# dfki-asr/morphablegraphs

Hardware: AMD Instinct MI355X
Metric: motion-primitive samples scored+back-projected/sec; fraction of HBM roofline (higher is better)
Workload: dtype f32; 1 GPU; walk primitive L=40 F=156 D=79 NB=31 GMM k=8, batch=8192 candidates/GPU (BASELINE.json configs[1]); candidates_per_gpu=8192, global_candidates=8192, collective=none, clock_ramp_steps=1500

## Files before the change

include/mg_hip.h:

```cpp
#ifndef MG_HIP_H
#define MG_HIP_H

#include <stdint.h>

#ifdef __cplusplus
extern "C" {
#endif

typedef struct mg_context mg_context;
typedef struct mg_primitive mg_primitive;
typedef struct mg_time_grid mg_time_grid;
typedef struct mg_constraint_set mg_constraint_set;

enum {
    MG_OK = 0,
    MG_ERR_INVALID_ARGUMENT = -1,
    MG_ERR_NO_DEVICE = -2,
    MG_ERR_HIP = -3,
    MG_ERR_UNSUPPORTED = -4,
    MG_ERR_NOT_POSITIVE_DEFINITE = -5,
    MG_ERR_OUT_OF_MEMORY = -6
};

enum { MG_F32 = 0, MG_F64 = 1 };
// ... 81 lines not shown
#define MG_OPT_FORCE_VALU_SCORE 0
#define MG_OPT_FORCE_VALU_SAMPLE 1
#define MG_OPT_RING_SLOTS 2
#define MG_OPT_CHUNK_WINDOW 3
#define MG_OPT_CHUNK_SAMPLES 4
#define MG_OPT_FRAMES_KERNEL 5
#define MG_OPT_PLACED_FAST_PCT 6
#define MG_OPT_OPTIONS_STEP 7
#define MG_OPT_PLAIN_MALLOC 8
#define MG_OPT_GMM_KERNEL 9
#define MG_OPT_SCORE_KERNEL 10
#define MG_OPT_ROOT_MODE 11
#define MG_OPT_PLACED_HOLD 12
#define MG_OPT_TRAJECTORY_LANES 13
#define MG_OPT_TRAJECTORY_SEARCH 14
#define MG_OPT_COUNT 15
int mg_context_set_option(mg_context *ctx, int32_t option, int32_t value);
int mg_context_arena_begin(mg_context *ctx, int64_t block_bytes);
int mg_context_arena_end(mg_context *ctx);
int mg_context_arena_bytes(mg_context *ctx, int64_t *reserved, int64_t *used);
int mg_context_synchronize(mg_context *ctx);
int mg_context_device_info(mg_context *ctx, char *name, int32_t *n_cu, int64_t *total_mem);

int mg_device_malloc(mg_context *ctx, int64_t bytes, void **out_dev);
int mg_device_free(mg_context *ctx, void *ptr_dev);
int mg_context_trim_outputs(mg_context *ctx);
int mg_context_output_bytes(mg_context *ctx, int64_t *reserved, int64_t *in_use, int32_t *n_regions, int32_t *n_fast);
int mg_device_malloc_chunked(mg_context *ctx, int64_t bytes, int64_t chunk_bytes, void **out_dev);
int mg_device_malloc_placed(mg_context *ctx, int64_t bytes, int32_t max_candidates, void **out_dev, double *info4);
int mg_device_probe_placement(mg_context *ctx, void *buf_dev, int64_t bytes, double *info4);
int mg_device_placement_info(mg_context *ctx, const void *buf_dev, double *info4, double *tbps);
// ... 317 lines not shown
```

morphablegraphs_amd/_capi.py:

```python
import ctypes as C
import functools
import itertools
import os

import numpy as np

HERE = os.path.dirname(os.path.abspath(__file__))
LIB_PATH = os.path.join(HERE, "csrc", "libmg_hip.so")

MG_OK = 0
MG_ERR_INVALID_ARGUMENT = -1
MG_ERR_UNSUPPORTED = -4
MG_F32, MG_F64 = 0, 1
MG_PATH_AUTO, MG_PATH_MFMA, MG_PATH_DIRECT = 0, 1, 2
MG_ALIGN_START_POSE = -1
MG_OPT_FORCE_VALU_SCORE, MG_OPT_FORCE_VALU_SAMPLE, MG_OPT_RING_SLOTS, MG_OPT_CHUNK_WINDOW, MG_OPT_CHUNK_SAMPLES = 0, 1, 2, 3, 4
MG_OPT_FRAMES_KERNEL = 5
MG_OPT_PLACED_FAST_PCT = 6
MG_OPT_OPTIONS_STEP = 7
MG_OPT_PLAIN_MALLOC = 8
MG_OPT_GMM_KERNEL = 9
MG_OPT_SCORE_KERNEL = 10
MG_OPT_ROOT_MODE = 11
MG_OPT_PLACED_HOLD = 12
MG_OPT_TRAJECTORY_LANES = 13
MG_OPT_TRAJECTORY_SEARCH = 14
MG_OPT_COUNT = 15
MG_CONSTRAINT_POSITION, MG_CONSTRAINT_DIRECTION_2D, MG_CONSTRAINT_JOINT_POSITION = 0, 1, 2
MG_CONSTRAINT_JOINT_MIDPOINT, MG_CONSTRAINT_JOINT_ORIENTATION, MG_CONSTRAINT_LOOK_AT, MG_CONSTRAINT_POSE = 3, 4, 5, 6
MG_CONSTRAINT_VALUE_POSITION, MG_CONSTRAINT_VALUE_HEADING = 7, 8
PROFILE_SLOTS = {"frames": 0, "gmm_log_prob": 1, "score_constraints": 2, "argmin": 3,
                 "gmm_sample": 4, "spline_evaluate": 5, "step": 6, "options_step": 7, "joint_tracks": 8, "frame_constraints": 9, "trajectory": 10,
                 "cluster_tree_search": 11, "walk_frames": 12}
MG_TREE_MAX_DEPTH, MG_TREE_MAX_CHILDREN, MG_TREE_MAX_CANDIDATES = 64, 256, 64
MG_TREE_TIE, MG_TREE_NO_RESULT, MG_TREE_OVERFLOW, MG_TREE_NO_MEAN = 1, 2, 4, 8
MG_KD_MAX_DEPTH = 64
TREE_SEARCH_RECORD = np.dtype([("row", "<i8"), ("leaf", "<i4"), ("flags", "<i4"), ("evaluations", "<i8"), ("value", "<f8")])
MG_WALK_MAX_STEPS = 64
MG_WALK_TILE = 32
MG_FUSED_MAX_OPTIONS = 24


# ... 1470 lines not shown
```

morphablegraphs_amd/csrc/mg_gmm.hip:

```cpp
#include <cstring>

#include <algorithm>

#include "mg_internal.h"
#include "mg_gmm_device.h"
#include "mg_score_device.h"

#define MG_GMM_CANDS 64
#define MG_GMM_WAVES 8

struct mg_gmm_args {
    const double *P;
    const double *mP;
    const double *cst;
    const void *x;
    void *out;
    int64_t B, ld;
    int32_t K, L;
};

template <bool X_F64, bool OUT_F64>
__global__ __launch_bounds__(MG_GMM_CANDS *MG_GMM_WAVES) void mg_gmm_logp_kernel(mg_gmm_args a) {
    extern __shared__ __attribute__((aligned(16))) unsigned char smem[];
    const int L = a.L, K = a.K;
// ... 131 lines not shown
    for (int q = 0; q < MG_JAC_ITEMS; q++) {
        const int e = tid + 256 * q;
        if (e < MG_JAC_CANDS * L) {
            const int c = e / L, i = e - c * L;
            if (c < ncand)
                ((double *)a.out)[(b0 + c) * L + i] = (exp(lds_lp[c]) == 0.0) ? 1.0 : g[q];
        }
    }
}



struct mg_gmm_mfma_args {
    int64_t B, ld;
    int32_t K, L, JT;
};

template <int KK, bool X_F64, bool OUT_F64>
__global__ __launch_bounds__(256) void mg_gmm_logp_mfma_kernel(const double *__restrict__ Ppack,
                                                              const double *__restrict__ mP,
                                                              const double *__restrict__ cst,
                                                              const void *__restrict__ x, void *__restrict__ out,
                                                              const mg_gmm_mfma_args a) {
    extern __shared__ __attribute__((aligned(16))) unsigned char smem[];
    mg_lds_f64 *lds_t = (mg_lds_f64 *)smem;
    mg_lds_f64 *lds_e = lds_t + a.K * 16;
    const int tid = threadIdx.x, lane = tid & 63;
    const int wave = __builtin_amdgcn_readfirstlane(tid >> 6);
    const int cl = lane & 15, g = lane >> 4;
    const int64_t b0 = (int64_t)blockIdx.x * 16;
    const int ncand = (int)((a.B - b0) < 16 ? (a.B - b0) : 16);
    typename mg_gmm_xt<X_F64>::type xf[KK];
    mg_gmm_load_x<KK, X_F64>(xf, x, b0, ncand, a.ld, a.L, cl, g);
    for (int k = wave; k < a.K; k += 4) {
        mg_gmm_frag<KK> f;
        mg_gmm_load_component<KK>(f, Ppack, mP, cst, k, a.JT, lane, cl, a.K);
        mg_gmm_apply_component(f, k, a.JT, xf, lds_t, cl, g);
    }
    __syncthreads();
    for (int e = tid; e < a.K * 16; e += 256) lds_e[e] = mg_gmm_exp_entry(lds_t, a.K, e);
    __syncthreads();
    if (tid < ncand) {
        const double r = mg_gmm_logsumexp(lds_t, lds_e, a.K, tid);
        if (OUT_F64) ((double *)out)[b0 + tid] = r;
        else ((float *)out)[b0 + tid] = (float)r;
    }
}

template <int KK>
static int mg_launch_gmm_mfma_kk(mg_primitive *p, const void *x, int xdt, int64_t B, int64_t ld, void *out, int odt) {
    mg_gmm_mfma_args a;
    a.B = B; a.ld = ld; a.K = p->K; a.L = p->Lg; a.JT = (p->Lg + 15) / 16;
    const int64_t grid = (B + 15) / 16;
    if (grid > 0x7fffffff) { mg_set_error("mg_gmm_log_prob: too many samples"); return MG_ERR_UNSUPPORTED; }
    const size_t lds = (size_t)p->K * 16 * 8 * 2;
    hipStream_t st = p->ctx->stream;
    const bool xf = xdt == MG_F64, of = odt == MG_F64;
    if (xf && of) hipLaunchKernelGGL((mg_gmm_logp_mfma_kernel<KK, true, true>), dim3((int)grid), dim3(256), lds, st, p->d_gPpack, p->d_gmPpad, p->d_gconst, x, out, a);
    else if (xf) hipLaunchKernelGGL((mg_gmm_logp_mfma_kernel<KK, true, false>), dim3((int)grid), dim3(256), lds, st, p->d_gPpack, p->d_gmPpad, p->d_gconst, x, out, a);
    else if (of) hipLaunchKernelGGL((mg_gmm_logp_mfma_kernel<KK, false, true>), dim3((int)grid), dim3(256), lds, st, p->d_gPpack, p->d_gmPpad, p->d_gconst, x, out, a);
    else hipLaunchKernelGGL((mg_gmm_logp_mfma_kernel<KK, false, false>), dim3((int)grid), dim3(256), lds, st, p->d_gPpack, p->d_gmPpad, p->d_gconst, x, out, a);
    MG_HIP_CHECK(hipGetLastError());
    return MG_OK;
}

template <int KK>
__host__ __device__ constexpr int mg_gmm_nf() {
    int nf = 0;
    for (int jt = 0; jt < (KK + 3) / 4; jt++) nf += (4 * (jt + 1) < KK) ? 4 * (jt + 1) : KK;
    return nf;
}
struct mg_objective_args {
    mg_score_args sa;
    const double *Wpack, *bpad;
    int32_t RT, rows, wave_doubles;
    int32_t pair_doubles;
    double error_scale, quality_scale;
    double *err_out, *obj_out;
};
template <bool SCORE> struct mg_gmm_lds_nw { static constexpr int value = SCORE ? 12 : 16; };
template <int KK, bool X_F64, bool OUT_F64, bool SCORE>
__global__ __launch_bounds__(64 * mg_gmm_lds_nw<SCORE>::value) void mg_gmm_logp_lds_kernel(const double *__restrict__ Ppack,
                                                               const double *__restrict__ mP,
                                                               const double *__restrict__ cst,
                                                               const void *__restrict__ x, void *__restrict__ out,
                                                               const mg_gmm_mfma_args a, const int64_t n_tiles, const mg_objective_args oa) {
    constexpr int JTM = (KK + 3) / 4;
    constexpr int NW = mg_gmm_lds_nw<SCORE>::value;
    extern __shared__ __attribute__((aligned(16))) unsigned char smem[];
    const int K = a.K;
    constexpr int JT = JTM;
    constexpr int nf = mg_gmm_nf<KK>();
    mg_lds_f64 *lds_f = (mg_lds_f64 *)smem;
    mg_lds_f64 *lds_c = lds_f + (size_t)K * nf * 64;
    mg_lds_f64 *lds_w = lds_c + (size_t)K * JT * 16;
    const int tid = threadIdx.x, lane = tid & 63;
    const int wave = __builtin_amdgcn_readfirstlane(tid >> 6);
    const int cl = lane & 15, g = lane >> 4;
    typedef double mg_f64x2 __attribute__((ext_vector_type(2)));
    const mg_f64x2 *P2 = (const mg_f64x2 *)(Ppack + (size_t)K * JT * KK * 64);
#pragma unroll 4
    for (int F2 = wave; F2 < K * nf / 2; F2 += NW) {
        const int F = 2 * F2, k = F / nf, f = F - k * nf;
        int jt = 0, off = 0;
#pragma unroll
        for (int j = 0; j < JTM - 1; j++) {
            const int n = (4 * (j + 1) < KK) ? 4 * (j + 1) : KK;
            if (f >= off + n) { off += n; jt = j + 1; }
        }
        const mg_f64x2 v = P2[(((size_t)k * JT + jt) * (KK / 2) + (f - off) / 2) * 64 + lane];
        lds_f[F * 64 + lane] = v[0];
        lds_f[(F + 1) * 64 + lane] = v[1];
    }
    for (int e = tid; e < K * JT * 16; e += 64 * NW) lds_c[e] = -mP[e];
    __syncthreads();
    mg_lds_f64 *terms = lds_w + (size_t)wave * (SCORE ? oa.wave_doubles : 2 * K * 16), *exps = terms + K * 16;
    double *vals_b = SCORE && oa.pair_doubles > 0 ? (double *)(lds_w + (size_t)NW * oa.wave_doubles + (size_t)wave * oa.pair_doubles) : nullptr;
    bool pending = false;
    double r_a = 0.0;
    int64_t b0_a = 0;
    int ncand_a = 0;
    for (int64_t tile = (int64_t)wave * gridDim.x + blockIdx.x; tile < n_tiles; tile += (int64_t)gridDim.x * NW) {
        const int64_t b0 = tile * 16;
        const int ncand = (int)((a.B - b0) < 16 ? (a.B - b0) : 16);
        typename mg_gmm_xt<X_F64>::type xf[KK];
        mg_gmm_load_x<KK, X_F64>(xf, x, b0, ncand, a.ld, a.L, cl, g);
        for (int k = 0; k < K; k++) {
            __builtin_amdgcn_sched_barrier(0);
            const mg_lds_f64 *fk = lds_f + (size_t)k * nf * 64 + lane;
            mg_f64x4 acc[JTM];
#pragma unroll
            for (int jt = 0; jt < JTM; jt++) {
                const double c0 = lds_c[(k * JT + jt) * 16 + cl];
                acc[jt] = {c0, c0, c0, c0};
            }
#pragma unroll
            for (int kk = 0; kk < KK; kk++) {
                int off = 0;
#pragma unroll
                for (int jt = 0; jt < JTM; jt++) {
                    if (kk < 4 * (jt + 1)) acc[jt] = __builtin_amdgcn_mfma_f64_16x16x4f64((double)xf[kk], fk[(off + kk) * 64], acc[jt], 0, 0, 0);
                    off += (4 * (jt + 1) < KK) ? 4 * (jt + 1) : KK;
                }
            }
// ... 70 lines not shown
#define MG_GMM_LDS_MIN_B 20480
static int mg_objective_wave_doubles(const mg_primitive *p, const mg_constraint_set *cs) {
    return std::max(2 * p->K * 16, 16 * (cs->rows + 1) + 32 * std::max(cs->n, 1));
}
template <int KK>
static int mg_launch_gmm_lds_kk(mg_primitive *p, const void *x, int xdt, int64_t B, int64_t ld, void *out, int odt,
                                const mg_constraint_set *cs = nullptr, double error_scale = 0.0, double quality_scale = 0.0,
                                double *err_out = nullptr, double *obj_out = nullptr) {
    mg_gmm_mfma_args a;
    a.B = B; a.ld = ld; a.K = p->K; a.L = p->Lg; a.JT = (p->Lg + 15) / 16;
    const int64_t n_tiles = (B + 15) / 16;
    mg_objective_args oa;
    memset(&oa, 0, sizeof(oa));
    const int wave_doubles = cs ? mg_objective_wave_doubles(p, cs) : 2 * p->K * 16;
    const int nw = cs ? mg_gmm_lds_nw<true>::value : mg_gmm_lds_nw<false>::value;
    size_t lds = ((size_t)p->K * mg_gmm_lds_nf(KK, a.JT) * 64 + (size_t)p->K * a.JT * 16 + (size_t)nw * wave_doubles) * 8;
    const int pair_doubles = cs ? 16 * (cs->rows + 1) : 0;
    const bool pairs = cs && lds + (size_t)nw * pair_doubles * 8 <= 160 * 1024;
    if (pairs) lds += (size_t)nw * pair_doubles * 8;
    if (cs) {
        mg_score_args &sa = oa.sa;
        sa = mg_score_args_of(cs, p->L);
        sa.lat = x; sa.B = B; sa.ld = ld;
        oa.Wpack = cs->d_Wpack; oa.bpad = cs->d_bpad; oa.RT = cs->RT; oa.rows = cs->rows; oa.wave_doubles = wave_doubles;
        oa.pair_doubles = pairs ? pair_doubles : 0;
        oa.error_scale = error_scale; oa.quality_scale = quality_scale; oa.err_out = err_out; oa.obj_out = obj_out;
    }
    const int grid = (int)std::min<int64_t>(std::max(1, p->ctx->n_cu), n_tiles);
    hipStream_t st = p->ctx->stream;
    const bool xf = xdt == MG_F64, of = odt == MG_F64;
    const unsigned abit = 1u << (KK / 2);
    if (!(p->ctx->attr_gmm_lds & abit)) {
        MG_HIP_CHECK(hipFuncSetAttribute((const void *)mg_gmm_logp_lds_kernel<KK, true, true, false>, hipFuncAttributeMaxDynamicSharedMemorySize, 160 * 1024));
        MG_HIP_CHECK(hipFuncSetAttribute((const void *)mg_gmm_logp_lds_kernel<KK, true, false, false>, hipFuncAttributeMaxDynamicSharedMemorySize, 160 * 1024));
        MG_HIP_CHECK(hipFuncSetAttribute((const void *)mg_gmm_logp_lds_kernel<KK, false, true, false>, hipFuncAttributeMaxDynamicSharedMemorySize, 160 * 1024));
        MG_HIP_CHECK(hipFuncSetAttribute((const void *)mg_gmm_logp_lds_kernel<KK, false, false, false>, hipFuncAttributeMaxDynamicSharedMemorySize, 160 * 1024));
        MG_HIP_CHECK(hipFuncSetAttribute((const void *)mg_gmm_logp_lds_kernel<KK, true, true, true>, hipFuncAttributeMaxDynamicSharedMemorySize, 160 * 1024));
        MG_HIP_CHECK(hipFuncSetAttribute((const void *)mg_gmm_logp_lds_kernel<KK, false, true, true>, hipFuncAttributeMaxDynamicSharedMemorySize, 160 * 1024));
        p->ctx->attr_gmm_lds |= abit;
    }
    if (cs) {
        if (xf) hipLaunchKernelGGL((mg_gmm_logp_lds_kernel<KK, true, true, true>), dim3(grid), dim3(64 * nw), lds, st, p->d_gPpack, p->d_gmPpad, p->d_gconst, x, out, a, n_tiles, oa);
        else hipLaunchKernelGGL((mg_gmm_logp_lds_kernel<KK, false, true, true>), dim3(grid), dim3(64 * nw), lds, st, p->d_gPpack, p->d_gmPpad, p->d_gconst, x, out, a, n_tiles, oa);
    }
    else if (xf && of) hipLaunchKernelGGL((mg_gmm_logp_lds_kernel<KK, true, true, false>), dim3(grid), dim3(1024), lds, st, p->d_gPpack, p->d_gmPpad, p->d_gconst, x, out, a, n_tiles, oa);
    else if (xf) hipLaunchKernelGGL((mg_gmm_logp_lds_kernel<KK, true, false, false>), dim3(grid), dim3(1024), lds, st, p->d_gPpack, p->d_gmPpad, p->d_gconst, x, out, a, n_tiles, oa);
    else if (of) hipLaunchKernelGGL((mg_gmm_logp_lds_kernel<KK, false, true, false>), dim3(grid), dim3(1024), lds, st, p->d_gPpack, p->d_gmPpad, p->d_gconst, x, out, a, n_tiles, oa);
    else hipLaunchKernelGGL((mg_gmm_logp_lds_kernel<KK, false, false, false>), dim3(grid), dim3(1024), lds, st, p->d_gPpack, p->d_gmPpad, p->d_gconst, x, out, a, n_tiles, oa);
    MG_HIP_CHECK(hipGetLastError());
    return MG_OK;
}

bool mg_objective_can_fuse(const mg_primitive *p, const mg_constraint_set *cs) {
    if (!p->d_gPpack || p->KKg <= 0 || p->Lg != p->L || p->KK != p->KKg || !cs || !cs->d_Wpack || p->ctx->opt[MG_OPT_FORCE_VALU_SCORE]) return false;
    for (const mg_keyframe_constraint &kc : cs->structure)
        if (kc.type != MG_CONSTRAINT_POSITION && kc.type != MG_CONSTRAINT_DIRECTION_2D) return false;
    if (cs->has_pose || cs->align_joint > 0) return false;
    const int JT = (p->Lg + 15) / 16;
    if (JT != (p->KKg + 3) / 4) return false;
    const size_t lds = ((size_t)p->K * mg_gmm_lds_nf(p->KKg, JT) * 64 + (size_t)p->K * JT * 16 + (size_t)mg_gmm_lds_nw<true>::value * mg_objective_wave_doubles(p, cs)) * 8;
    return lds <= 160 * 1024 - 64;
}
int mg_launch_objective(mg_primitive *p, const mg_constraint_set *cs, const void *x, int xdt, int64_t B, int64_t ld, double error_scale,
// ... 440 lines not shown
```

morphablegraphs_amd/csrc/mg_gmm_device.h:

```cpp
#pragma once
#include <hip/hip_runtime.h>

#include <cmath>

typedef double mg_f64x4 __attribute__((ext_vector_type(4)));
typedef __attribute__((address_space(3))) double mg_lds_f64;
typedef __attribute__((address_space(3))) float mg_lds_f32;

template <bool X_F64> struct mg_gmm_xt { typedef double type; };
template <> struct mg_gmm_xt<false> { typedef float type; };

template <int KK, bool X_F64>
__device__ __forceinline__ void mg_gmm_load_x(typename mg_gmm_xt<X_F64>::type (&xf)[KK], const void *x, int64_t b0, int ncand,
                                              int64_t ld, int L, int cl, int g) {
    typedef typename mg_gmm_xt<X_F64>::type T;
    const int c = cl < ncand ? cl : ncand - 1;
    const bool rok = cl < ncand;
    const T *row = (const T *)x + (b0 + c) * ld;
    const T *rowg = row + g;
#pragma unroll
    for (int kk = 0; kk < KK; kk++) {
        if (kk < KK - 2) {
            const T v = rowg[4 * kk];
            xf[kk] = rok ? v : (T)0;
// ... 57 lines not shown
template <int JTM>
__device__ __forceinline__ void mg_gmm_finish_component(const mg_f64x4 (&acc)[JTM], int JT, double cst, int k, mg_lds_f64 *terms, int cl, int g) {
    double part[4] = {0.0, 0.0, 0.0, 0.0};
#pragma unroll
    for (int jt = 0; jt < JTM; jt++)
        if (jt < JT) {
#pragma unroll
            for (int r = 0; r < 4; r++) part[r] = fma(acc[jt][r], acc[jt][r], part[r]);
        }
#pragma unroll
    for (int r = 0; r < 4; r++) part[r] = mg_row16_sum(part[r]);
    if (cl == 0) {
#pragma unroll
        for (int r = 0; r < 4; r++) terms[k * 16 + g + 4 * r] = cst - 0.5 * part[r];
    }
}

template <int KK, typename T, bool WIDEN_AT_USE = false>
__device__ __forceinline__ void mg_gmm_apply_component(const mg_gmm_frag<KK> &f, int k, int JT, const T (&xf)[KK],
                                                       mg_lds_f64 *terms, int cl, int g) {
    constexpr int JTM = mg_gmm_frag<KK>::JTM;
    mg_f64x4 acc[JTM];
#pragma unroll
    for (int jt = 0; jt < JTM; jt++) acc[jt] = {f.c0[jt], f.c0[jt], f.c0[jt], f.c0[jt]};
#pragma unroll
    for (int kk = 0; kk < KK; kk++) {
        T xv = xf[kk];
        if constexpr (WIDEN_AT_USE) asm volatile("" : "+v"(xv));
        const double xd = (double)xv;
#pragma unroll
// ... 104 lines not shown
```

morphablegraphs_amd/csrc/mg_host.hip:

```cpp
#include <algorithm>
#include <cmath>
#include <cstdarg>
#include <cstdio>
#include <cstdlib>
#include <cstring>
#include <new>
#include <time.h>

#include "mg_internal.h"
#include <dlfcn.h>

static thread_local char g_err[1024] = "";

void mg_set_error(const char *fmt, ...) {
    va_list ap;
    va_start(ap, fmt);
    vsnprintf(g_err, sizeof(g_err), fmt, ap);
    va_end(ap);
}

int mg_hip_fail(hipError_t e, const char *what) {
    mg_set_error("HIP error %d (%s) in %s", (int)e, hipGetErrorString(e), what);
    if (e == hipErrorOutOfMemory) return MG_ERR_OUT_OF_MEMORY;
    if (e == hipErrorNoDevice || e == hipErrorInvalidDevice) return MG_ERR_NO_DEVICE;
// ... 80 lines not shown
        return MG_ERR_UNSUPPORTED;
    }
    if (stream) {
        ctx->stream = (hipStream_t)stream;
        ctx->own_stream = false;
    } else {
        e = hipStreamCreateWithFlags(&ctx->stream, hipStreamNonBlocking);
        if (e != hipSuccess) { delete ctx; return mg_hip_fail(e, "hipStreamCreate"); }
        ctx->own_stream = true;
    }
    e = hipMalloc(&ctx->argmin_out, 16);
    if (e != hipSuccess) { mg_context_destroy(ctx); return mg_hip_fail(e, "hipMalloc"); }
    int rc = mg_setup_kernel_attributes(ctx);
    if (rc == MG_OK) rc = mg_options_fused_attributes();
    if (rc != MG_OK) { mg_context_destroy(ctx); return rc; }
    *out = ctx;
    return MG_OK;
}

static void mg_vmm_release(mg_context *ctx, mg_context::vmm_alloc &v);
extern "C" void mg_context_destroy(mg_context *ctx) {
    if (!ctx) return;
    (void)hipSetDevice(ctx->device);
    (void)hipStreamSynchronize(ctx->stream);
    if (ctx->rccl_comm && g_rccl.CommDestroy) { (void)g_rccl.CommDestroy(ctx->rccl_comm); ctx->rccl_comm = nullptr; }
    for (auto &p : ctx->pending) { (void)hipEventDestroy(p.a); (void)hipEventDestroy(p.b); }
    for (auto &ev : ctx->free_events) (void)hipEventDestroy(ev);
    for (auto &st : ctx->side) if (st) (void)hipStreamDestroy(st);
    for (auto &e : ctx->side_ev) if (e) (void)hipEventDestroy(e);
    if (ctx->scratch) (void)mg_device_free(ctx, ctx->scratch);
// ... 147 lines not shown
    ctx->dist_rank = 0; ctx->dist_ranks = 1;
    return nrc == 0 ? MG_OK : mg_rccl_fail(nrc, "ncclCommDestroy");
}

extern "C" int mg_context_synchronize(mg_context *ctx) {
    MG_REQUIRE(ctx != nullptr, "mg_context_synchronize: ctx is NULL");
    MG_HIP_CHECK(hipStreamSynchronize(ctx->stream));
    return MG_OK;
}

extern "C" int mg_context_set_reserved_cus(mg_context *ctx, int32_t n) {
    MG_REQUIRE(ctx != nullptr && n >= 0, "mg_context_set_reserved_cus: bad arguments");
    ctx->reserved_cus = std::min<int32_t>(n, ctx->n_cu - 1);
    return MG_OK;
}
extern "C" int mg_context_set_option(mg_context *ctx, int32_t option, int32_t value) {
    MG_REQUIRE(ctx != nullptr, "mg_context_set_option: ctx is NULL");
    MG_REQUIRE(option >= 0 && option < MG_OPT_COUNT, "mg_context_set_option: unknown option %d", option);
    MG_REQUIRE(value >= 0, "mg_context_set_option: value %d < 0", value);
    ctx->opt[option] = value;
    return MG_OK;
}
extern "C" int mg_context_device_info(mg_context *ctx, char *name, int32_t *n_cu, int64_t *total_mem) {
    MG_REQUIRE(ctx != nullptr, "mg_context_device_info: ctx is NULL");
    if (name) { strncpy(name, ctx->name, 255); name[255] = 0; }
    if (n_cu) *n_cu = ctx->n_cu;
    if (total_mem) *total_mem = ctx->total_mem;
    return MG_OK;
}

// ... 440 lines not shown
extern "C" mg_time_grid *mg_primitive_canonical_grid(mg_primitive *prim) { return prim ? prim->canonical : nullptr; }
extern "C" int mg_time_grid_size(const mg_time_grid *g) { return g ? g->T : 0; }
extern "C" int mg_time_grid_get_tables(const mg_time_grid *g, int32_t *i0, double *weights, double *times) {
    MG_REQUIRE(g != nullptr, "mg_time_grid_get_tables: grid is NULL");
    if (i0) std::copy(g->i0.begin(), g->i0.end(), i0);
    if (weights) std::copy(g->w.begin(), g->w.end(), weights);
    if (times) std::copy(g->times.begin(), g->times.end(), times);
    return MG_OK;
}

static void mg_primitive_free(mg_primitive *p) {
    if (!p) return;
    (void)hipSetDevice(p->ctx->device);
    (void)hipStreamSynchronize(p->ctx->stream);
    void *ptrs[] = {p->d_Epack, p->d_Et32, p->d_Et64, p->d_Erpack, p->d_meanroot, p->d_mean32, p->d_mean, p->d_knots,
                    p->d_gP, p->d_gmP, p->d_gconst, p->d_gmean, p->d_gchol, p->d_gPpack, p->d_gmPpad, p->d_gPTpack, p->d_gcholpack, p->d_gmeanpad,
                    p->d_tphi, p->d_tmean};
    for (void *q : ptrs) mg_dev_free(p->ctx, q);
    for (mg_time_grid *g : {p->canonical, p->coeff_grid})
        if (g) { mg_free_grid_device(g); delete g; }
    delete p;
}

extern "C" void mg_primitive_destroy(mg_primitive *p) {
    if (p && p->ctx) p->ctx->fused_next.valid = false;
    mg_primitive_free(p);
}

extern "C" int mg_primitive_create(mg_context *ctx, const mg_primitive_desc *d, mg_primitive **out) {
    MG_REQUIRE(ctx && d && out, "mg_primitive_create: NULL argument");
    *out = nullptr;
// ... 197 lines not shown
            if (rc == MG_OK) rc = mg_upload(ctx, cpack, &p->d_gcholpack);
            if (rc == MG_OK) rc = mg_upload(ctx, meanpad, &p->d_gmeanpad);
            {
                const size_t n1 = ppack.size();
                ppack.resize(2 * n1, 0.0);
                for (int k = 0; k < K; k++)
                    for (int jt = 0; jt < JT; jt++)
                        for (int q = 0; q < KK / 2; q++)
                            for (int lane = 0; lane < 64; lane++)
                                for (int h = 0; h < 2; h++)
                                    ppack[n1 + ((((size_t)k * JT + jt) * (KK / 2) + q) * 64 + lane) * 2 + h] = ppack[((((size_t)k * JT + jt) * KK) + 2 * q + h) * 64 + lane];
            }
            if (rc == MG_OK) rc = mg_upload(ctx, ppack, &p->d_gPpack);
            if (rc == MG_OK) rc = mg_upload(ctx, ptpack, &p->d_gPTpack);
            if (rc == MG_OK) rc = mg_upload(ctx, mpad, &p->d_gmPpad);
        }
        if (rc == MG_OK) rc = mg_upload(ctx, gP, &p->d_gP);
        if (rc == MG_OK) rc = mg_upload(ctx, gmP, &p->d_gmP);
        if (rc == MG_OK) rc = mg_upload(ctx, gconst, &p->d_gconst);
        if (rc == MG_OK) rc = mg_upload(ctx, p->gm, &p->d_gmean);
        if (rc == MG_OK) rc = mg_upload(ctx, chol, &p->d_gchol);
        if (rc != MG_OK) { mg_primitive_free(p); return rc; }
    }

    {
        std::vector<double> m2(L, 1.0);
        double wsum = 0.0;
        for (int j = 0; j < K; j++) wsum += p->gw[j];
        if (K > 0)
            for (int k = 0; k < L; k++) {
// ... 1189 lines not shown
```

morphablegraphs_amd/csrc/mg_internal.h:

```cpp
#pragma once
#include <hip/hip_runtime.h>

#include <cstdint>
#include <map>
#include <string>
#include <vector>

#include "../../include/mg_hip.h"

#define MG_NCAND 16
#define MG_ROWTILE 16
#define MG_MAX_KK 16
#define MG_BLOCK 256
#define MG_PROFILE_SLOTS 13

void mg_set_error(const char *fmt, ...);
int mg_hip_fail(hipError_t e, const char *what);

#define MG_HIP_CHECK(expr)                                   \
    do {                                                     \
        hipError_t _e = (expr);                              \
        if (_e != hipSuccess) return mg_hip_fail(_e, #expr); \
    } while (0)

#define MG_REQUIRE_AS(cond, code, ...) \
    do {                               \
        if (!(cond)) {                 \
            mg_set_error(__VA_ARGS__); \
            return (code);             \
        }                              \
    } while (0)

struct mg_event_pair {
    hipEvent_t a, b;
    int slot;
    bool ended;
    int slot2 = -1;
};

struct mg_context {
    int device = 0;
    hipStream_t stream = nullptr;
    bool own_stream = false;
    int n_cu = 0;
    int64_t total_mem = 0;
    int max_lds = 0;
    char name[256] = {0};
    bool profile = false;
    std::vector<mg_event_pair> pending;
    std::vector<hipEvent_t> free_events;
    int reserved_cus = 0;
    int32_t opt[MG_OPT_COUNT] = {0};
    int prof_interval = 1;
// ... 119 lines not shown
    std::vector<double> knots;
    std::vector<double> gw, gm, gc, gp;
    int32_t Dp = 0;
    int32_t cshift = 0;
    float *d_Epack = nullptr;
    float *d_Et32 = nullptr;
    double *d_Et64 = nullptr;
    double *d_Erpack = nullptr;
    double *d_meanroot = nullptr;
    float *d_mean32 = nullptr;
    double *d_mean = nullptr;
    double *d_knots = nullptr;
    int32_t RRT = 0;
    double *d_gPpack = nullptr;
    double *d_gmPpad = nullptr;
    double *d_gP = nullptr;
    double *d_gmP = nullptr;
    double *d_gPTpack = nullptr;
    double *d_gcholpack = nullptr;
    double *d_gmeanpad = nullptr;
    double *d_gconst = nullptr;
    double *d_gmean = nullptr;
    double *d_gchol = nullptr;
    mg_time_grid *canonical = nullptr;
    mg_time_grid *coeff_grid = nullptr;
};

struct mg_constraint_set {
    mg_primitive *prim = nullptr;
    int32_t n = 0;
// ... 106 lines not shown
```

Before: 106.5 million samples/s.

## Pack half-empty last GMM precision tiles of component pairs into one MFMA tile

When the latent width leaves the last 16-column tile of each component's Cholesky-like precision matrix at most half full, a host-side image now packs two components' last tiles into one shared 16-wide tile. The MFMA and LDS GMM log-prob kernels then run a single MFMA chain for that tile per component pair and split the result with a DPP swap. This removes MFMA work and LDS fragment storage spent on zero-padded columns. The cost is extra index arithmetic in the fragment staging loop, more code paths, and one extra device buffer. It is enabled by default through a new context option.

```diff
diff --git a/include/mg_hip.h b/include/mg_hip.h
--- a/include/mg_hip.h
+++ b/include/mg_hip.h
@@ -119,7 +119,8 @@
 #define MG_OPT_PLACED_HOLD 12
 #define MG_OPT_TRAJECTORY_LANES 13
 #define MG_OPT_TRAJECTORY_SEARCH 14
-#define MG_OPT_COUNT 15
+#define MG_OPT_GMM_PACK_LAST 15
+#define MG_OPT_COUNT 16
 int mg_context_set_option(mg_context *ctx, int32_t option, int32_t value);
 int mg_context_arena_begin(mg_context *ctx, int64_t block_bytes);
 int mg_context_arena_end(mg_context *ctx);
diff --git a/morphablegraphs_amd/_capi.py b/morphablegraphs_amd/_capi.py
--- a/morphablegraphs_amd/_capi.py
+++ b/morphablegraphs_amd/_capi.py
@@ -25,7 +25,8 @@
 MG_OPT_PLACED_HOLD = 12
 MG_OPT_TRAJECTORY_LANES = 13
 MG_OPT_TRAJECTORY_SEARCH = 14
-MG_OPT_COUNT = 15
+MG_OPT_GMM_PACK_LAST = 15
+MG_OPT_COUNT = 16
 MG_CONSTRAINT_POSITION, MG_CONSTRAINT_DIRECTION_2D, MG_CONSTRAINT_JOINT_POSITION = 0, 1, 2
 MG_CONSTRAINT_JOINT_MIDPOINT, MG_CONSTRAINT_JOINT_ORIENTATION, MG_CONSTRAINT_LOOK_AT, MG_CONSTRAINT_POSE = 3, 4, 5, 6
 MG_CONSTRAINT_VALUE_POSITION, MG_CONSTRAINT_VALUE_HEADING = 7, 8
diff --git a/morphablegraphs_amd/csrc/mg_gmm.hip b/morphablegraphs_amd/csrc/mg_gmm.hip
--- a/morphablegraphs_amd/csrc/mg_gmm.hip
+++ b/morphablegraphs_amd/csrc/mg_gmm.hip
@@ -169,10 +169,14 @@
 struct mg_gmm_mfma_args {
     int64_t B, ld;
     int32_t K, L, JT;
+    int32_t pack;
 };
+
+static bool mg_gmm_pack_last(const mg_primitive *p) { return p->d_gPshare != nullptr && p->ctx->opt[MG_OPT_GMM_PACK_LAST] != 0; }
 
 template <int KK, bool X_F64, bool OUT_F64>
 __global__ __launch_bounds__(256) void mg_gmm_logp_mfma_kernel(const double *__restrict__ Ppack,
+                                                              const double *__restrict__ Pshare,
                                                               const double *__restrict__ mP,
                                                               const double *__restrict__ cst,
                                                               const void *__restrict__ x, void *__restrict__ out,
@@ -187,10 +191,29 @@
     const int ncand = (int)((a.B - b0) < 16 ? (a.B - b0) : 16);
     typename mg_gmm_xt<X_F64>::type xf[KK];
     mg_gmm_load_x<KK, X_F64>(xf, x, b0, ncand, a.ld, a.L, cl, g);
-    for (int k = wave; k < a.K; k += 4) {
-        mg_gmm_frag<KK> f;
-        mg_gmm_load_component<KK>(f, Ppack, mP, cst, k, a.JT, lane, cl, a.K);
-        mg_gmm_apply_component(f, k, a.JT, xf, lds_t, cl, g);
+    bool packed = false;
+    if constexpr (mg_gmm_packable<KK>::value) packed = a.pack != 0;
+    if (packed) {
+        if constexpr (mg_gmm_packable<KK>::value) {
+            for (int u = wave; 2 * u < a.K; u += 4) {
+                const int k = 2 * u;
+                if (k + 1 < a.K) {
+                    mg_gmm_pair_frag<KK> f;
+                    mg_gmm_load_pair<KK>(f, Ppack, Pshare, mP, cst, k, lane, cl, a.K);
+                    mg_gmm_apply_pair(f, k, xf, lds_t, cl, g);
+                } else {
+                    mg_gmm_frag<KK> f;
+                    mg_gmm_load_component<KK>(f, Ppack, mP, cst, k, a.JT, lane, cl, a.K);
+                    mg_gmm_apply_component(f, k, a.JT, xf, lds_t, cl, g);
+                }
+            }
+        }
+    } else {
+        for (int k = wave; k < a.K; k += 4) {
+            mg_gmm_frag<KK> f;
+            mg_gmm_load_component<KK>(f, Ppack, mP, cst, k, a.JT, lane, cl, a.K);
+            mg_gmm_apply_component(f, k, a.JT, xf, lds_t, cl, g);
+        }
     }
     __syncthreads();
     for (int e = tid; e < a.K * 16; e += 256) lds_e[e] = mg_gmm_exp_entry(lds_t, a.K, e);
@@ -206,15 +229,16 @@
 static int mg_launch_gmm_mfma_kk(mg_primitive *p, const void *x, int xdt, int64_t B, int64_t ld, void *out, int odt) {
     mg_gmm_mfma_args a;
     a.B = B; a.ld = ld; a.K = p->K; a.L = p->Lg; a.JT = (p->Lg + 15) / 16;
+    a.pack = mg_gmm_packable<KK>::value && mg_gmm_pack_last(p) ? 1 : 0;
     const int64_t grid = (B + 15) / 16;
     if (grid > 0x7fffffff) { mg_set_error("mg_gmm_log_prob: too many samples"); return MG_ERR_UNSUPPORTED; }
     const size_t lds = (size_t)p->K * 16 * 8 * 2;
     hipStream_t st = p->ctx->stream;
     const bool xf = xdt == MG_F64, of = odt == MG_F64;
-    if (xf && of) hipLaunchKernelGGL((mg_gmm_logp_mfma_kernel<KK, true, true>), dim3((int)grid), dim3(256), lds, st, p->d_gPpack, p->d_gmPpad, p->d_gconst, x, out, a);
-    else if (xf) hipLaunchKernelGGL((mg_gmm_logp_mfma_kernel<KK, true, false>), dim3((int)grid), dim3(256), lds, st, p->d_gPpack, p->d_gmPpad, p->d_gconst, x, out, a);
-    else if (of) hipLaunchKernelGGL((mg_gmm_logp_mfma_kernel<KK, false, true>), dim3((int)grid), dim3(256), lds, st, p->d_gPpack, p->d_gmPpad, p->d_gconst, x, out, a);
-    else hipLaunchKernelGGL((mg_gmm_logp_mfma_kernel<KK, false, false>), dim3((int)grid), dim3(256), lds, st, p->d_gPpack, p->d_gmPpad, p->d_gconst, x, out, a);
+    if (xf && of) hipLaunchKernelGGL((mg_gmm_logp_mfma_kernel<KK, true, true>), dim3((int)grid), dim3(256), lds, st, p->d_gPpack, p->d_gPshare, p->d_gmPpad, p->d_gconst, x, out, a);
+    else if (xf) hipLaunchKernelGGL((mg_gmm_logp_mfma_kernel<KK, true, false>), dim3((int)grid), dim3(256), lds, st, p->d_gPpack, p->d_gPshare, p->d_gmPpad, p->d_gconst, x, out, a);
+    else if (of) hipLaunchKernelGGL((mg_gmm_logp_mfma_kernel<KK, false, true>), dim3((int)grid), dim3(256), lds, st, p->d_gPpack, p->d_gPshare, p->d_gmPpad, p->d_gconst, x, out, a);
+    else hipLaunchKernelGGL((mg_gmm_logp_mfma_kernel<KK, false, false>), dim3((int)grid), dim3(256), lds, st, p->d_gPpack, p->d_gPshare, p->d_gmPpad, p->d_gconst, x, out, a);
     MG_HIP_CHECK(hipGetLastError());
     return MG_OK;
 }
@@ -236,6 +260,7 @@
 template <bool SCORE> struct mg_gmm_lds_nw { static constexpr int value = SCORE ? 12 : 16; };
 template <int KK, bool X_F64, bool OUT_F64, bool SCORE>
 __global__ __launch_bounds__(64 * mg_gmm_lds_nw<SCORE>::value) void mg_gmm_logp_lds_kernel(const double *__restrict__ Ppack,
+                                                               const double *__restrict__ Pshare,
                                                                const double *__restrict__ mP,
                                                                const double *__restrict__ cst,
                                                                const void *__restrict__ x, void *__restrict__ out,
@@ -246,28 +271,44 @@
     const int K = a.K;
     constexpr int JT = JTM;
     constexpr int nf = mg_gmm_nf<KK>();
+    constexpr int nfull = nf - KK, nfp = 2 * nfull + KK;
+    bool packed = false;
+    if constexpr (mg_gmm_packable<KK>::value) packed = a.pack != 0;
+    const int NP = packed ? K / 2 : 0, n_frag = packed ? NP * nfp + (K & 1) * nf : K * nf;
     mg_lds_f64 *lds_f = (mg_lds_f64 *)smem;
-    mg_lds_f64 *lds_c = lds_f + (size_t)K * nf * 64;
-    mg_lds_f64 *lds_w = lds_c + (size_t)K * JT * 16;
+    mg_lds_f64 *lds_c = lds_f + (size_t)n_frag * 64;
+    mg_lds_f64 *lds_cs = lds_c + (size_t)K * JT * 16;
+    mg_lds_f64 *lds_w = lds_cs + (size_t)NP * 16;
     const int tid = threadIdx.x, lane = tid & 63;
     const int wave = __builtin_amdgcn_readfirstlane(tid >> 6);
     const int cl = lane & 15, g = lane >> 4;
     typedef double mg_f64x2 __attribute__((ext_vector_type(2)));
     const mg_f64x2 *P2 = (const mg_f64x2 *)(Ppack + (size_t)K * JT * KK * 64);
 #pragma unroll 4
-    for (int F2 = wave; F2 < K * nf / 2; F2 += NW) {
-        const int F = 2 * F2, k = F / nf, f = F - k * nf;
+    for (int F2 = wave; F2 < n_frag / 2; F2 += NW) {
+        const int F = 2 * F2;
+        int k = F / nf, f = F - k * nf;
+        const mg_f64x2 *src = P2;
+        if (packed) {
+            const int j = F / nfp, fp = F - j * nfp;
+            if (j >= NP) { k = K - 1; f = F - NP * nfp; }
+            else if (fp < nfull) { k = 2 * j; f = fp; }
+            else if (fp < 2 * nfull) { k = 2 * j + 1; f = fp - nfull; }
+            else { src = (const mg_f64x2 *)Pshare + ((size_t)j * (KK / 2) + (fp - 2 * nfull) / 2) * 64; k = -1; }
+        }
         int jt = 0, off = 0;
 #pragma unroll
         for (int j = 0; j < JTM - 1; j++) {
             const int n = (4 * (j + 1) < KK) ? 4 * (j + 1) : KK;
             if (f >= off + n) { off += n; jt = j + 1; }
         }
-        const mg_f64x2 v = P2[(((size_t)k * JT + jt) * (KK / 2) + (f - off) / 2) * 64 + lane];
+        if (k >= 0) src = P2 + (((size_t)k * JT + jt) * (KK / 2) + (f - off) / 2) * 64;
+        const mg_f64x2 v = src[lane];
         lds_f[F * 64 + lane] = v[0];
         lds_f[(F + 1) * 64 + lane] = v[1];
     }
     for (int e = tid; e < K * JT * 16; e += 64 * NW) lds_c[e] = -mP[e];
+    for (int e = tid; e < NP * 16; e += 64 * NW) lds_cs[e] = -(Pshare + (size_t)NP * KK * 64)[e];
     __syncthreads();
     mg_lds_f64 *terms = lds_w + (size_t)wave * (SCORE ? oa.wave_doubles : 2 * K * 16), *exps = terms + K * 16;
     double *vals_b = SCORE && oa.pair_doubles > 0 ? (double *)(lds_w + (size_t)NW * oa.wave_doubles + (size_t)wave * oa.pair_doubles) : nullptr;
@@ -280,9 +321,61 @@
         const int ncand = (int)((a.B - b0) < 16 ? (a.B - b0) : 16);
         typename mg_gmm_xt<X_F64>::type xf[KK];
         mg_gmm_load_x<KK, X_F64>(xf, x, b0, ncand, a.ld, a.L, cl, g);
-        for (int k = 0; k < K; k++) {
+        if constexpr (mg_gmm_packable<KK>::value) {
+            for (int j = 0; j < NP; j++) {
+                __builtin_amdgcn_sched_barrier(0);
+                const mg_lds_f64 *fa = lds_f + (size_t)j * nfp * 64 + lane, *fb = fa + nfull * 64, *fs = fb + nfull * 64;
+                double pa[4], pb[4], ya[4], yb[4];
+                {
+                    mg_f64x4 acc[JTM];
+#pragma unroll
+                    for (int jt = 0; jt < JTM - 1; jt++) {
+                        const double c0 = lds_c[(2 * j * JT + jt) * 16 + cl];
+                        acc[jt] = {c0, c0, c0, c0};
+                    }
+#pragma unroll
+                    for (int kk = 0; kk < KK; kk++) {
+                        int off = 0;
+#pragma unroll
+                        for (int jt = 0; jt < JTM - 1; jt++) {
+                            if (kk < 4 * (jt + 1)) acc[jt] = __builtin_amdgcn_mfma_f64_16x16x4f64((double)xf[kk], fa[(off + kk) * 64], acc[jt], 0, 0, 0);
+                            off += 4 * (jt + 1);
+                        }
+                    }
+                    mg_gmm_square_full_tiles<JTM>(acc, pa);
+                }
+                {
+                    const double c0 = lds_cs[j * 16 + cl];
+                    mg_f64x4 accs = {c0, c0, c0, c0};
+#pragma unroll
+                    for (int kk = 0; kk < KK; kk++) accs = __builtin_amdgcn_mfma_f64_16x16x4f64((double)xf[kk], fs[kk * 64], accs, 0, 0, 0);
+                    mg_gmm_split_shared_tile(accs, cl, ya, yb);
+                }
+                mg_gmm_finish_parts(pa, ya, cst[2 * j], 2 * j, terms, cl, g);
+                {
+                    mg_f64x4 acc[JTM];
+#pragma unroll
+                    for (int jt = 0; jt < JTM - 1; jt++) {
+                        const double c0 = lds_c[((2 * j + 1) * JT + jt) * 16 + cl];
+                        acc[jt] = {c0, c0, c0, c0};
+                    }
+#pragma unroll
+                    for (int kk = 0; kk < KK; kk++) {
+                        int off = 0;
+#pragma unroll
+                        for (int jt = 0; jt < JTM - 1; jt++) {
+                            if (kk < 4 * (jt + 1)) acc[jt] = __builtin_amdgcn_mfma_f64_16x16x4f64((double)xf[kk], fb[(off + kk) * 64], acc[jt], 0, 0, 0);
+                            off += 4 * (jt + 1);
+                        }
+                    }
+                    mg_gmm_square_full_tiles<JTM>(acc, pb);
+                }
+                mg_gmm_finish_parts(pb, yb, cst[2 * j + 1], 2 * j + 1, terms, cl, g);
+            }
+        }
+        for (int k = 2 * NP; k < K; k++) {
             __builtin_amdgcn_sched_barrier(0);
-            const mg_lds_f64 *fk = lds_f + (size_t)k * nf * 64 + lane;
+            const mg_lds_f64 *fk = lds_f + ((size_t)NP * nfp + (size_t)(k - 2 * NP) * nf) * 64 + lane;
             mg_f64x4 acc[JTM];
 #pragma unroll
             for (int jt = 0; jt < JTM; jt++) {
@@ -383,7 +476,9 @@
     memset(&oa, 0, sizeof(oa));
     const int wave_doubles = cs ? mg_objective_wave_doubles(p, cs) : 2 * p->K * 16;
     const int nw = cs ? mg_gmm_lds_nw<true>::value : mg_gmm_lds_nw<false>::value;
-    size_t lds = ((size_t)p->K * mg_gmm_lds_nf(KK, a.JT) * 64 + (size_t)p->K * a.JT * 16 + (size_t)nw * wave_doubles) * 8;
+    a.pack = mg_gmm_packable<KK>::value && mg_gmm_pack_last(p) ? 1 : 0;
+    const size_t n_frag = (size_t)p->K * mg_gmm_lds_nf(KK, a.JT) - (a.pack ? (size_t)(p->K / 2) * KK : 0);
+    size_t lds = (n_frag * 64 + (size_t)p->K * a.JT * 16 + (a.pack ? (size_t)(p->K / 2) * 16 : 0) + (size_t)nw * wave_doubles) * 8;
     const int pair_doubles = cs ? 16 * (cs->rows + 1) : 0;
     const bool pairs = cs && lds + (size_t)nw * pair_doubles * 8 <= 160 * 1024;
     if (pairs) lds += (size_t)nw * pair_doubles * 8;
@@ -409,13 +504,13 @@
         p->ctx->attr_gmm_lds |= abit;
     }
     if (cs) {
-        if (xf) hipLaunchKernelGGL((mg_gmm_logp_lds_kernel<KK, true, true, true>), dim3(grid), dim3(64 * nw), lds, st, p->d_gPpack, p->d_gmPpad, p->d_gconst, x, out, a, n_tiles, oa);
-        else hipLaunchKernelGGL((mg_gmm_logp_lds_kernel<KK, false, true, true>), dim3(grid), dim3(64 * nw), lds, st, p->d_gPpack, p->d_gmPpad, p->d_gconst, x, out, a, n_tiles, oa);
-    }
-    else if (xf && of) hipLaunchKernelGGL((mg_gmm_logp_lds_kernel<KK, true, true, false>), dim3(grid), dim3(1024), lds, st, p->d_gPpack, p->d_gmPpad, p->d_gconst, x, out, a, n_tiles, oa);
-    else if (xf) hipLaunchKernelGGL((mg_gmm_logp_lds_kernel<KK, true, false, false>), dim3(grid), dim3(1024), lds, st, p->d_gPpack, p->d_gmPpad, p->d_gconst, x, out, a, n_tiles, oa);
-    else if (of) hipLaunchKernelGGL((mg_gmm_logp_lds_kernel<KK, false, true, false>), dim3(grid), dim3(1024), lds, st, p->d_gPpack, p->d_gmPpad, p->d_gconst, x, out, a, n_tiles, oa);
-    else hipLaunchKernelGGL((mg_gmm_logp_lds_kernel<KK, false, false, false>), dim3(grid), dim3(1024), lds, st, p->d_gPpack, p->d_gmPpad, p->d_gconst, x, out, a, n_tiles, oa);
+        if (xf) hipLaunchKernelGGL((mg_gmm_logp_lds_kernel<KK, true, true, true>), dim3(grid), dim3(64 * nw), lds, st, p->d_gPpack, p->d_gPshare, p->d_gmPpad, p->d_gconst, x, out, a, n_tiles, oa);
+        else hipLaunchKernelGGL((mg_gmm_logp_lds_kernel<KK, false, true, true>), dim3(grid), dim3(64 * nw), lds, st, p->d_gPpack, p->d_gPshare, p->d_gmPpad, p->d_gconst, x, out, a, n_tiles, oa);
+    }
+    else if (xf && of) hipLaunchKernelGGL((mg_gmm_logp_lds_kernel<KK, true, true, false>), dim3(grid), dim3(1024), lds, st, p->d_gPpack, p->d_gPshare, p->d_gmPpad, p->d_gconst, x, out, a, n_tiles, oa);
+    else if (xf) hipLaunchKernelGGL((mg_gmm_logp_lds_kernel<KK, true, false, false>), dim3(grid), dim3(1024), lds, st, p->d_gPpack, p->d_gPshare, p->d_gmPpad, p->d_gconst, x, out, a, n_tiles, oa);
+    else if (of) hipLaunchKernelGGL((mg_gmm_logp_lds_kernel<KK, false, true, false>), dim3(grid), dim3(1024), lds, st, p->d_gPpack, p->d_gPshare, p->d_gmPpad, p->d_gconst, x, out, a, n_tiles, oa);
+    else hipLaunchKernelGGL((mg_gmm_logp_lds_kernel<KK, false, false, false>), dim3(grid), dim3(1024), lds, st, p->d_gPpack, p->d_gPshare, p->d_gmPpad, p->d_gconst, x, out, a, n_tiles, oa);
     MG_HIP_CHECK(hipGetLastError());
     return MG_OK;
 }
diff --git a/morphablegraphs_amd/csrc/mg_gmm_device.h b/morphablegraphs_amd/csrc/mg_gmm_device.h
--- a/morphablegraphs_amd/csrc/mg_gmm_device.h
+++ b/morphablegraphs_amd/csrc/mg_gmm_device.h
@@ -95,6 +95,110 @@
 #pragma unroll
         for (int r = 0; r < 4; r++) terms[k * 16 + g + 4 * r] = cst - 0.5 * part[r];
     }
+}
+
+template <int KK> struct mg_gmm_packable { static constexpr bool value = (KK % 4 == 2) && KK <= 10; };
+
+template <int JTM>
+__device__ __forceinline__ void mg_gmm_square_full_tiles(const mg_f64x4 (&acc)[JTM], double (&part)[4]) {
+#pragma unroll
+    for (int r = 0; r < 4; r++) part[r] = 0.0;
+#pragma unroll
+    for (int jt = 0; jt < JTM - 1; jt++) {
+#pragma unroll
+        for (int r = 0; r < 4; r++) part[r] = fma(acc[jt][r], acc[jt][r], part[r]);
+    }
+}
+__device__ __forceinline__ void mg_gmm_split_shared_tile(const mg_f64x4 &accs, int cl, double (&ya)[4], double (&yb)[4]) {
+    const bool lo = cl < 8;
+#pragma unroll
+    for (int r = 0; r < 4; r++) {
+        const double s = accs[r];
+        const double m = mg_dpp_f64<0x128>(s);
+        ya[r] = lo ? s : 0.0;
+        yb[r] = lo ? m : 0.0;
+    }
+}
+__device__ __forceinline__ void mg_gmm_finish_parts(double (&part)[4], const double (&ylast)[4], double cst, int k, mg_lds_f64 *terms, int cl, int g) {
+#pragma unroll
+    for (int r = 0; r < 4; r++) part[r] = mg_row16_sum(fma(ylast[r], ylast[r], part[r]));
+    if (cl == 0) {
+#pragma unroll
+        for (int r = 0; r < 4; r++) terms[k * 16 + g + 4 * r] = cst - 0.5 * part[r];
+    }
+}
+
+template <int KK>
+struct mg_gmm_pair_frag {
+    static constexpr int JTM = (KK + 3) / 4;
+    double pfa[JTM][KK], pfb[JTM][KK], pfs[KK];
+    double c0a[JTM], c0b[JTM], c0s;
+    double csta, cstb;
+};
+template <int KK>
+__device__ __forceinline__ void mg_gmm_load_pair(mg_gmm_pair_frag<KK> &f, const double *__restrict__ Ppack, const double *__restrict__ Pshare,
+                                                 const double *__restrict__ mP, const double *__restrict__ cst, int k, int lane, int cl, int K) {
+    typedef double mg_f64x2 __attribute__((ext_vector_type(2)));
+    constexpr int JTM = mg_gmm_pair_frag<KK>::JTM;
+    const mg_f64x2 *P2 = (const mg_f64x2 *)(Ppack + (size_t)K * JTM * KK * 64);
+#pragma unroll
+    for (int jt = 0; jt < JTM - 1; jt++) {
+        const mg_f64x2 *pa = P2 + (((size_t)k * JTM + jt) * (KK / 2)) * 64 + lane;
+        const mg_f64x2 *pb = pa + (size_t)JTM * (KK / 2) * 64;
+#pragma unroll
+        for (int q = 0; q < KK / 2; q++)
+            if (2 * q < 4 * (jt + 1)) {
+                const mg_f64x2 va = pa[q * 64], vb = pb[q * 64];
+                f.pfa[jt][2 * q] = va[0]; f.pfa[jt][2 * q + 1] = va[1];
+                f.pfb[jt][2 * q] = vb[0]; f.pfb[jt][2 * q + 1] = vb[1];
+            }
+        f.c0a[jt] = -mP[((size_t)k * JTM + jt) * 16 + cl];
+        f.c0b[jt] = -mP[((size_t)(k + 1) * JTM + jt) * 16 + cl];
+    }
+    const mg_f64x2 *ps = (const mg_f64x2 *)Pshare + ((size_t)(k / 2) * (KK / 2)) * 64 + lane;
+#pragma unroll
+    for (int q = 0; q < KK / 2; q++) {
+        const mg_f64x2 v = ps[q * 64];
+        f.pfs[2 * q] = v[0]; f.pfs[2 * q + 1] = v[1];
+    }
+    f.c0s = -(Pshare + (size_t)(K / 2) * KK * 64)[(k / 2) * 16 + cl];
+    f.csta = cst[k];
+    f.cstb = cst[k + 1];
+}
+template <int KK, typename T>
+__device__ __forceinline__ void mg_gmm_apply_pair(const mg_gmm_pair_frag<KK> &f, int k, const T (&xf)[KK], mg_lds_f64 *terms, int cl, int g) {
+    constexpr int JTM = mg_gmm_pair_frag<KK>::JTM;
+    double pa[4], pb[4], ya[4], yb[4];
+    {
+        mg_f64x4 acc[JTM];
+#pragma unroll
+        for (int jt = 0; jt < JTM - 1; jt++) acc[jt] = {f.c0a[jt], f.c0a[jt], f.c0a[jt], f.c0a[jt]};
+#pragma unroll
+        for (int kk = 0; kk < KK; kk++)
+#pragma unroll
+            for (int jt = 0; jt < JTM - 1; jt++)
+                if (kk < 4 * (jt + 1)) acc[jt] = __builtin_amdgcn_mfma_f64_16x16x4f64((double)xf[kk], f.pfa[jt][kk], acc[jt], 0, 0, 0);
+        mg_gmm_square_full_tiles<JTM>(acc, pa);
+    }
+    {
+        mg_f64x4 accs = {f.c0s, f.c0s, f.c0s, f.c0s};
+#pragma unroll
+        for (int kk = 0; kk < KK; kk++) accs = __builtin_amdgcn_mfma_f64_16x16x4f64((double)xf[kk], f.pfs[kk], accs, 0, 0, 0);
+        mg_gmm_split_shared_tile(accs, cl, ya, yb);
+    }
+    mg_gmm_finish_parts(pa, ya, f.csta, k, terms, cl, g);
+    {
+        mg_f64x4 acc[JTM];
+#pragma unroll
+        for (int jt = 0; jt < JTM - 1; jt++) acc[jt] = {f.c0b[jt], f.c0b[jt], f.c0b[jt], f.c0b[jt]};
+#pragma unroll
+        for (int kk = 0; kk < KK; kk++)
+#pragma unroll
+            for (int jt = 0; jt < JTM - 1; jt++)
+                if (kk < 4 * (jt + 1)) acc[jt] = __builtin_amdgcn_mfma_f64_16x16x4f64((double)xf[kk], f.pfb[jt][kk], acc[jt], 0, 0, 0);
+        mg_gmm_square_full_tiles<JTM>(acc, pb);
+    }
+    mg_gmm_finish_parts(pb, yb, f.cstb, k + 1, terms, cl, g);
 }
 
 template <int KK, typename T, bool WIDEN_AT_USE = false>
diff --git a/morphablegraphs_amd/csrc/mg_host.hip b/morphablegraphs_amd/csrc/mg_host.hip
--- a/morphablegraphs_amd/csrc/mg_host.hip
+++ b/morphablegraphs_amd/csrc/mg_host.hip
@@ -118,6 +118,7 @@
     int rc = mg_setup_kernel_attributes(ctx);
     if (rc == MG_OK) rc = mg_options_fused_attributes();
     if (rc != MG_OK) { mg_context_destroy(ctx); return rc; }
+    ctx->opt[MG_OPT_GMM_PACK_LAST] = 1;
     *out = ctx;
     return MG_OK;
 }
@@ -295,6 +296,29 @@
     ctx->reserved_cus = std::min<int32_t>(n, ctx->n_cu - 1);
     return MG_OK;
 }
+extern "C" int64_t mg_gmm_pack_last_tiles(const double *P, const double *mP, int32_t K, int32_t Lg, int32_t KK, double *image, int64_t capacity) {
+    MG_REQUIRE(P && mP && K >= 1 && Lg >= 1 && KK >= 2 && KK % 2 == 0 && 4 * KK >= Lg, "mg_gmm_pack_last_tiles: bad arguments");
+    const int rem = Lg % 16, NP = K / 2;
+    if (rem < 1 || rem > 8 || NP < 1) return 0;
+    const int64_t n = (int64_t)NP * KK * 64 + (int64_t)NP * 16;
+    if (!image) return n;
+    MG_REQUIRE(capacity >= n, "mg_gmm_pack_last_tiles: capacity %lld < %lld", (long long)capacity, (long long)n);
+    std::fill(image, image + n, 0.0);
+    const int j0 = 16 * ((Lg + 15) / 16 - 1);
+    double *mrow = image + (size_t)NP * KK * 64;
+    for (int pr = 0; pr < NP; pr++)
+        for (int c = 0; c < 16; c++) {
+            const int k = 2 * pr + (c >> 3), j = j0 + (c & 7);
+            if (j >= Lg) continue;
+            mrow[pr * 16 + c] = mP[(size_t)k * Lg + j];
+            for (int kk = 0; kk < KK; kk++)
+                for (int gq = 0; gq < 4; gq++) {
+                    const int i = 4 * kk + gq, lane = 16 * gq + c;
+                    if (i < Lg && i <= j) image[(((size_t)pr * (KK / 2) + kk / 2) * 64 + lane) * 2 + (kk & 1)] = P[((size_t)k * Lg + i) * Lg + j];
+                }
+        }
+    return n;
+}
 extern "C" int mg_context_set_option(mg_context *ctx, int32_t option, int32_t value) {
     MG_REQUIRE(ctx != nullptr, "mg_context_set_option: ctx is NULL");
     MG_REQUIRE(option >= 0 && option < MG_OPT_COUNT, "mg_context_set_option: unknown option %d", option);
@@ -765,7 +789,7 @@
     (void)hipSetDevice(p->ctx->device);
     (void)hipStreamSynchronize(p->ctx->stream);
     void *ptrs[] = {p->d_Epack, p->d_Et32, p->d_Et64, p->d_Erpack, p->d_meanroot, p->d_mean32, p->d_mean, p->d_knots,
-                    p->d_gP, p->d_gmP, p->d_gconst, p->d_gmean, p->d_gchol, p->d_gPpack, p->d_gmPpad, p->d_gPTpack, p->d_gcholpack, p->d_gmeanpad,
+                    p->d_gP, p->d_gmP, p->d_gconst, p->d_gmean, p->d_gchol, p->d_gPpack, p->d_gmPpad, p->d_gPshare, p->d_gPTpack, p->d_gcholpack, p->d_gmeanpad,
                     p->d_tphi, p->d_tmean};
     for (void *q : ptrs) mg_dev_free(p->ctx, q);
     for (mg_time_grid *g : {p->canonical, p->coeff_grid})
@@ -993,6 +1017,12 @@
             if (rc == MG_OK) rc = mg_upload(ctx, ppack, &p->d_gPpack);
             if (rc == MG_OK) rc = mg_upload(ctx, ptpack, &p->d_gPTpack);
             if (rc == MG_OK) rc = mg_upload(ctx, mpad, &p->d_gmPpad);
+            const int64_t n_share = mg_gmm_pack_last_tiles(p->gp.data(), gmP.data(), K, Lg, KK, nullptr, 0);
+            if (n_share > 0 && JT == (KK + 3) / 4) {
+                std::vector<double> share((size_t)n_share);
+                mg_gmm_pack_last_tiles(p->gp.data(), gmP.data(), K, Lg, KK, share.data(), n_share);
+                if (rc == MG_OK) rc = mg_upload(ctx, share, &p->d_gPshare);
+            }
         }
         if (rc == MG_OK) rc = mg_upload(ctx, gP, &p->d_gP);
         if (rc == MG_OK) rc = mg_upload(ctx, gmP, &p->d_gmP);
diff --git a/morphablegraphs_amd/csrc/mg_internal.h b/morphablegraphs_amd/csrc/mg_internal.h
--- a/morphablegraphs_amd/csrc/mg_internal.h
+++ b/morphablegraphs_amd/csrc/mg_internal.h
@@ -37,6 +37,8 @@
     bool ended;
     int slot2 = -1;
 };
+
+extern "C" int64_t mg_gmm_pack_last_tiles(const double *P, const double *mP, int32_t K, int32_t Lg, int32_t KK, double *image, int64_t capacity);
 
 struct mg_context {
     int device = 0;
@@ -186,6 +188,7 @@
     int32_t RRT = 0;
     double *d_gPpack = nullptr;
     double *d_gmPpad = nullptr;
+    double *d_gPshare = nullptr;
     double *d_gP = nullptr;
     double *d_gmP = nullptr;
     double *d_gPTpack = nullptr;
```

Measured after the change: 107.1 million samples/s (median of 5 runs). About the same (+0.5%).
